# scroll-tech/scroll-prover

Measured on NVIDIA H100. Metric: chunk-proof wall-sec (degree-26 SRS: k=20+24+25 replay), lower is better.
Workload: dtype u32x8 (254-bit Montgomery integers)

## Files before the change

scroll-prover_b200/csrc/msm.cu:

```cuda
#include "common.cuh"
#include "ec.cuh"

namespace b200zk {

static constexpr uint32_t PART_INVALID = 0x1fffffffu;
static constexpr uint32_t PART_GIANT = 0x20000000u;
static constexpr uint32_t PART_STARTS = 0x80000000u;
static constexpr uint32_t PART_ENDS = 0x40000000u;
static constexpr int MSM_MAX_BATCH = 32;
static constexpr int ACC_L_DEFAULT = 256;

struct MsmPlan {
    uint32_t c, W, B;
    uint32_t Ws;
    uint32_t batch;
    uint64_t stride;
    uint64_t NB;
};

struct MsmCols {
    const Fr* p[MSM_MAX_BATCH];
};

__device__ __forceinline__ void ld_affine(const Affine* p, Fq& x, Fq& y) {
// ... 507 lines not shown
__global__ void __launch_bounds__(128) msm_combine_heads(const uint32_t* __restrict__ part_id, const XYZZ* __restrict__ part_val,
                                                         uint64_t nrec, XYZZ* __restrict__ buckets) {
    uint64_t r = (uint64_t)blockIdx.x * blockDim.x + threadIdx.x;
    if (r >= nrec) return;
    uint32_t id = part_id[r];
    if ((id & PART_INVALID) == PART_INVALID || (id & PART_GIANT) || !(id & PART_STARTS)) return;
    XYZZ sum = ld_xyzz(part_val + r);
    uint64_t k = r;
    while (!(id & PART_ENDS)) {
        ++k;
        if (k >= nrec) break;
        id = part_id[k];
        if ((id & PART_INVALID) == PART_INVALID) { id = 0; continue; }
        XYZZ v = ld_xyzz(part_val + k);
        xyzz_add(sum, v);
    }
    st_xyzz(buckets + (part_id[r] & PART_INVALID), sum);
}

static constexpr int COMBINE_LR = 64;
__global__ void __launch_bounds__(128) msm_combine_level(const uint32_t* __restrict__ in_id, const XYZZ* __restrict__ in_val,
                                                         uint64_t nrec, XYZZ* __restrict__ buckets, uint32_t* __restrict__ out_id,
                                                         XYZZ* __restrict__ out_val, uint64_t nthreads,
                                                         const uint32_t* __restrict__ giant_flag) {
    if (*giant_flag == 0) return;
    uint64_t sigma = (uint64_t)blockIdx.x * blockDim.x + threadIdx.x;
    if (sigma >= nthreads) return;
    out_id[2 * sigma] = PART_INVALID;
    out_id[2 * sigma + 1] = PART_INVALID;
    uint64_t r0 = sigma * COMBINE_LR, r1 = r0 + COMBINE_LR;
    if (r1 > nrec) r1 = nrec;
    bool have = false;
    uint32_t cur = 0, flags = 0, slot = 0;
    XYZZ acc = XYZZ::identity();
    auto flush = [&]() {
        if (!have) return;
        if ((flags & PART_STARTS) && (flags & PART_ENDS)) {
            st_xyzz(buckets + cur, acc);
        } else {
            out_id[2 * sigma + slot] = cur | flags | PART_GIANT;
            st_xyzz(out_val + 2 * sigma + slot, acc);
            ++slot;
        }
    };
    for (uint64_t r = r0; r < r1; ++r) {
        uint32_t id = in_id[r];
        if ((id & PART_INVALID) == PART_INVALID || !(id & PART_GIANT)) continue;
        uint32_t bkt = id & PART_INVALID;
        if (!have || bkt != cur) {
            flush();
            have = true;
            cur = bkt;
            flags = id & (PART_STARTS | PART_ENDS);
            acc = ld_xyzz(in_val + r);
        } else {
            flags |= id & (PART_STARTS | PART_ENDS);
            XYZZ v = ld_xyzz(in_val + r);
            xyzz_add(acc, v);
        }
    }
    flush();
}

__global__ void __launch_bounds__(128) msm_combine_final(const uint32_t* __restrict__ part_id, const XYZZ* __restrict__ part_val,
                                                         uint64_t nrec, XYZZ* __restrict__ buckets, const uint32_t* __restrict__ giant_flag) {
    if (*giant_flag == 0) return;
    uint64_t r = (uint64_t)blockIdx.x * blockDim.x + threadIdx.x;
    if (r >= nrec) return;
    uint32_t id = part_id[r];
    if ((id & PART_INVALID) == PART_INVALID || !(id & PART_GIANT) || !(id & PART_STARTS)) return;
    XYZZ sum = ld_xyzz(part_val + r);
    uint64_t k = r;
    while (!(id & PART_ENDS)) {
        ++k;
        if (k >= nrec) break;
        id = part_id[k];
        if ((id & PART_INVALID) == PART_INVALID || !(id & PART_GIANT)) { id = 0; continue; }
        XYZZ v = ld_xyzz(part_val + k);
        xyzz_add(sum, v);
    }
    st_xyzz(buckets + (part_id[r] & PART_INVALID), sum);
}

static constexpr int RED_T = 128;

__device__ __forceinline__ void block_tree_sum(XYZZ& v, XYZZ* sh) {
    st_xyzz(sh + threadIdx.x, v);
    __syncthreads();
    for (uint32_t s = blockDim.x >> 1; s > 0; s >>= 1) {
        if (threadIdx.x < s) {
            XYZZ a = ld_xyzz(sh + threadIdx.x), b = ld_xyzz(sh + threadIdx.x + s);
            xyzz_add(a, b);
            st_xyzz(sh + threadIdx.x, a);
        }
        __syncthreads();
    }
    v = ld_xyzz(sh);
}

__global__ void __launch_bounds__(RED_T, 4) msm_rowcol_sums(const XYZZ* __restrict__ buckets, uint32_t B, uint32_t kc, XYZZ* __restrict__ vec) {
    __shared__ XYZZ sh[RED_T];
    const uint32_t cols = 1u << kc, rows = B >> kc;
    const XYZZ* bk = buckets + (uint64_t)blockIdx.y * B;
    XYZZ acc = XYZZ::identity();
    if (blockIdx.x < rows) {
        const XYZZ* r = bk + (uint64_t)blockIdx.x * cols;
        for (uint32_t lo = threadIdx.x; lo < cols; lo += blockDim.x) {
            XYZZ v = ld_xyzz(r + lo);
            xyzz_add(acc, v);
        }
    } else {
        uint32_t lo = blockIdx.x - rows;
        for (uint32_t hi = threadIdx.x; hi < rows; hi += blockDim.x) {
            XYZZ v = ld_xyzz(bk + (uint64_t)hi * cols + lo);
            xyzz_add(acc, v);
        }
    }
    block_tree_sum(acc, sh);
    if (threadIdx.x == 0) st_xyzz(vec + (uint64_t)blockIdx.y * (rows + cols) + blockIdx.x, acc);
}

__global__ void __launch_bounds__(RED_T, 4) msm_bit_sums(const XYZZ* __restrict__ vec, uint32_t B, uint32_t kc, uint32_t q_max,
                                                         XYZZ* __restrict__ out) {
    __shared__ XYZZ sh[RED_T];
    const uint32_t cols = 1u << kc, rows = B >> kc;
    const uint32_t which = blockIdx.y, b = blockIdx.x;
    const uint32_t m = which == 0 ? rows : cols;
    const XYZZ* v = vec + (uint64_t)blockIdx.z * (rows + cols) + (which == 0 ? 0 : rows);
    XYZZ acc = XYZZ::identity();
    const bool total = (b == q_max);
    if (total ? (which == 0) : ((1u << b) < m)) {
        for (uint32_t j = threadIdx.x; j < m; j += blockDim.x)
            if (total || ((j >> b) & 1u)) {
                XYZZ e = ld_xyzz(v + j);
                xyzz_add(acc, e);
            }
    }
    block_tree_sum(acc, sh);
    if (threadIdx.x == 0) st_xyzz(out + ((uint64_t)blockIdx.z * 2 + which) * (q_max + 1) + b, acc);
}

__global__ void __launch_bounds__(64) msm_finish(MsmPlan pl, uint32_t kc, uint32_t q_max, const XYZZ* __restrict__ bits_all, Jacobian* out_all) {
    __shared__ XYZZ ws[2];
    const uint32_t cols = 1u << kc, rows = pl.B >> kc;
    const uint32_t warp = threadIdx.x >> 5, lane = threadIdx.x & 31;
    Jacobian* out = out_all + blockIdx.x;
    XYZZ acc = XYZZ::identity();
    for (uint32_t w = pl.Ws; w-- > 0;) {
        const uint64_t set = (uint64_t)blockIdx.x * pl.Ws + w;
        const XYZZ* bits = bits_all + set * 2 * (q_max + 1);
        if (lane == 0) {
            const uint32_t m = warp == 0 ? rows : cols;
            const XYZZ* bv = bits + (uint64_t)warp * (q_max + 1);
            XYZZ h = XYZZ::identity();
            uint32_t q = 0;
            while ((1u << q) < m) ++q;
            for (uint32_t b = q; b-- > 0;) {
                if (!h.is_identity()) h = xyzz_dbl(h);
                XYZZ e = ld_xyzz(bv + b);
                xyzz_add(h, e);
            }
            st_xyzz(ws + warp, h);
        }
        __syncthreads();
        if (threadIdx.x == 0) {
            if (!acc.is_identity())
                for (uint32_t d = 0; d < pl.c; ++d) acc = xyzz_dbl(acc);
            XYZZ s = ld_xyzz(ws);
            for (uint32_t d = 0; d < kc; ++d) s = xyzz_dbl(s);
            XYZZ t = ld_xyzz(bits + q_max), u = ld_xyzz(ws + 1);
            xyzz_add(s, t);
            xyzz_add(s, u);
            xyzz_add(acc, s);
        }
        __syncthreads();
    }
    if (threadIdx.x == 0) *out = xyzz_to_jacobian_normalized(acc);
}

__global__ void g1_sum_kernel(const Jacobian* pts, uint64_t count, Jacobian* out) {
    if (threadIdx.x || blockIdx.x) return;
    XYZZ acc = XYZZ::identity();
    for (uint64_t i = 0; i < count; ++i) {
        XYZZ p = xyzz_from_jacobian(pts[i]);
        xyzz_add(acc, p);
    }
    *out = xyzz_to_jacobian_normalized(acc);
}

__global__ void __launch_bounds__(128) g1_generator_mul_kernel(const Fr* scalars, uint64_t n, Affine* out) {
    uint64_t i = (uint64_t)blockIdx.x * blockDim.x + threadIdx.x;
    if (i >= n) return;
    Fr s = scalars[i].from_mont();
    Fq gx = Fq::one(), gy = Fq::one().dbl();
    XYZZ acc = XYZZ::identity();
    for (int limb = 7; limb >= 0; --limb)
        for (int b = 31; b >= 0; --b) {
            acc = xyzz_dbl(acc);
            if ((s.l.v[limb] >> b) & 1) xyzz_madd(acc, gx, gy);
        }
    out[i] = xyzz_to_affine(acc);
}

static uint32_t pick_window(uint64_t n) {
    if (n < 32) return n < 4 ? 2 : 4;
    double best = 1e300;
    uint32_t bc = 8;
    for (uint32_t c = 5; c <= 23; ++c) {
        uint32_t W = 254 / c + 1;
        if ((double)n * W >= 4.0e9) continue;
        double cost = (double)n * W * 10.0 + (double)W * (double)(1ull << c) * 40.0 + (double)W * 4096.0;
        if (cost < best) {
            best = cost;
            bc = c;
        }
    }
    return bc;
}

static size_t align_up(size_t v, size_t a) { return (v + a - 1) / a * a; }

__global__ void __launch_bounds__(128) srs_shift_kernel(const Affine* __restrict__ in, Affine* __restrict__ out, uint64_t n, uint32_t c) {
    uint64_t i = (uint64_t)blockIdx.x * blockDim.x + threadIdx.x;
    if (i >= n) return;
    Affine a = in[i];
    XYZZ p = xyzz_from_affine(a);
    for (uint32_t d = 0; d < c; ++d) p = xyzz_dbl(p);
    out[i] = xyzz_to_affine(p);
}

static uint32_t pick_window_precomputed(uint64_t n) {
    double best = 1e300;
    uint32_t bc = 10;
    for (uint32_t c = 8; c <= 23; ++c) {
        uint32_t W = 254 / c + 1;
        if ((double)n * W >= 2.0e9) continue;
        double cost = (double)n * W * 10.0 + (double)(1ull << c) * 40.0;
        if (cost < best) {
            best = cost;
            bc = c;
        }
    }
    return bc;
}

static int32_t srs_precompute_run(b200zk_ctx* ctx, Affine* tables, uint64_t n, uint32_t c, uint32_t W) {
    for (uint32_t w = 1; w < W; ++w) {
        srs_shift_kernel<<<(uint32_t)((n + 127) / 128), 128, 0, ctx->stream>>>(tables + (uint64_t)(w - 1) * n, tables + (uint64_t)w * n, n, c);
        B2_LAUNCH_CHECK(ctx);
    }
    return B200ZK_OK;
}

static uint32_t msm_max_batch(uint64_t n, uint32_t pre_c) {
    uint32_t c = pre_c ? pre_c : pick_window(n);
    uint64_t per_col = (n ? n : 1) * (254 / c + 1);
    uint64_t b = (1ull << 28) / per_col;
    return (uint32_t)(b < 1 ? 1 : (b > MSM_MAX_BATCH ? MSM_MAX_BATCH : b));
}

static int32_t msm_run_batch(b200zk_ctx* ctx, const Affine* bases, const Fr* const* cols, uint32_t batch, uint64_t n, Jacobian* out_dev,
                             uint32_t pre_c, uint64_t pre_stride) {
    if (n >= (1ull << 31)) return fail(ctx, B200ZK_E_UNSUPPORTED, "msm: n = %llu >= 2^31", (unsigned long long)n);
    if (batch < 1 || batch > (uint32_t)MSM_MAX_BATCH) return fail(ctx, B200ZK_E_INVALID, "msm: batch %u out of range [1,%d]", batch, MSM_MAX_BATCH);
    MsmPlan pl;
    pl.c = pre_c ? pre_c : (ctx->msm_window ? ctx->msm_window : pick_window(n));
    if (pl.c < 2 || pl.c > 24) return fail(ctx, B200ZK_E_INVALID, "msm: window %u out of range [2,24]", pl.c);
    pl.W = 254 / pl.c + 1;
    pl.B = 1u << (pl.c - 1);
    pl.Ws = pre_c ? 1 : pl.W;
    pl.batch = batch;
    pl.stride = pre_c ? pre_stride : 0;
    pl.NB = (uint64_t)batch * pl.Ws * pl.B;
    uint64_t max_entries = n * pl.W * batch;
    if (max_entries >= 0xffffffffull) return fail(ctx, B200ZK_E_UNSUPPORTED, "msm: n*W*batch too large for window %u", pl.c);
    MsmCols colp;
    for (int q = 0; q < MSM_MAX_BATCH; ++q) colp.p[q] = cols[q < (int)batch ? q : 0];
    ctx->last_c = pl.c;
    ctx->last_windows = pl.W;
    ctx->last_adds = n * pl.W;

    const uint32_t ACC_L = ctx->msm_acc_l ? ctx->msm_acc_l : (uint32_t)ACC_L_DEFAULT;
    uint64_t nthreads = (max_entries + ACC_L - 1) / ACC_L;
    if (nthreads == 0) nthreads = 1;
    SortPlan sp;
    sp.FB = pl.c - 1 < SORT_FB_MAX ? pl.c - 1 : SORT_FB_MAX;
    sp.K = pl.B >> sp.FB;
    sp.wpg = pl.Ws == 1 ? pl.W : (COUNT_LOCAL_MAX / sp.K < 1 ? 1 : (COUNT_LOCAL_MAX / sp.K < pl.W ? COUNT_LOCAL_MAX / sp.K : pl.W));
    const uint32_t groups = (pl.W + sp.wpg - 1) / sp.wpg;
    const uint64_t nbins = pl.NB >> sp.FB;
    const uint32_t F = 1u << sp.FB;
    const uint64_t max_big = max_entries / SORT_BIG + 1;
    uint32_t ntiles = (uint32_t)((nbins + SCAN_TILE - 1) / SCAN_TILE);
    size_t off = 0;
    auto carve = [&](size_t bytes) { size_t o = off; off = align_up(off + bytes, 256); return o; };
    size_t o_offs = carve(4 * (pl.NB + 1));
    size_t o_bcnt = carve(4 * (nbins + 1)), o_boff = carve(4 * (nbins + 1)), o_bcur = carve(4 * (nbins + 1));
    size_t o_big = carve(4 * (max_big + 1)), o_bigc = carve(4 * 2 * F * max_big);
    size_t o_tiles = carve(4 * (size_t)(ntiles + 1));
    size_t o_flag = carve(256);
    size_t o_entries = carve(4 * (max_entries + 4));
    size_t o_digits = carve(4 * (max_entries + 4));
    size_t o_buckets = carve(sizeof(XYZZ) * pl.NB);
    size_t pval_bytes = sizeof(XYZZ) * 2 * nthreads;
    size_t o_pid = carve(4 * 2 * nthreads), o_pval = carve(pval_bytes > max_entries + 16 ? pval_bytes : max_entries + 16);
    uint64_t nthreads2 = (2 * nthreads + COMBINE_LR - 1) / COMBINE_LR;
    size_t o_pid2 = carve(4 * 2 * nthreads2), o_pval2 = carve(sizeof(XYZZ) * 2 * nthreads2);
    const uint32_t kc = pl.c / 2;
    const uint32_t red_cols = 1u << kc, red_rows = pl.B >> kc;
    const uint32_t sets = batch * pl.Ws;
    size_t red_len = (size_t)sets * (red_rows + red_cols);
    uint32_t q_max = 0;
    while ((1u << q_max) < (red_rows > red_cols ? red_rows : red_cols)) ++q_max;
    size_t o_gr = carve(sizeof(XYZZ) * red_len), o_sums = carve(sizeof(XYZZ) * 2 * (q_max + 1) * sets);
    B2_TRY(scratch_reserve(ctx, ctx->msm_work, off));
    char* base = (char*)ctx->msm_work.p;
    uint32_t* offsets = (uint32_t*)(base + o_offs);
    uint32_t* bin_cnt = (uint32_t*)(base + o_bcnt);
    uint32_t* bin_off = (uint32_t*)(base + o_boff);
    uint32_t* bin_cur = (uint32_t*)(base + o_bcur);
    uint32_t* big_list = (uint32_t*)(base + o_big);
    uint32_t* big_cnt = (uint32_t*)(base + o_bigc);
    uint32_t* tiles = (uint32_t*)(base + o_tiles);
    uint32_t* giant_flag = (uint32_t*)(base + o_flag);
    uint32_t* staged = (uint32_t*)(base + o_entries);
    uint32_t* digits = (uint32_t*)(base + o_digits);
    uint32_t* entries = digits;
    uint32_t* pid2 = (uint32_t*)(base + o_pid2);
    XYZZ* pval2 = (XYZZ*)(base + o_pval2);
    XYZZ* buckets = (XYZZ*)(base + o_buckets);
    uint32_t* pid = (uint32_t*)(base + o_pid);
    XYZZ* pval = (XYZZ*)(base + o_pval);
    uint8_t* fine = (uint8_t*)(base + o_pval);
    XYZZ* grpR = (XYZZ*)(base + o_gr);
    XYZZ* red_sums = (XYZZ*)(base + o_sums);

    cudaStream_t st = ctx->stream;
    B2_CUDA(ctx, cudaMemsetAsync(bin_cnt, 0, 4 * (nbins + 1), st));
    B2_CUDA(ctx, cudaMemsetAsync(big_list, 0, o_tiles - o_big, st));
    B2_CUDA(ctx, cudaMemsetAsync(giant_flag, 0, 4, st));
    B2_CUDA(ctx, cudaMemsetAsync(buckets, 0, sizeof(XYZZ) * pl.NB, st));
    const size_t count_smem = 4ull * (pl.Ws == 1 ? 1u : sp.wpg) * sp.K;
    const size_t part_smem = sp.K > PART_STAGE_K ? 4ull * sp.K : 4ull * (2 * sp.K + 2 * PART_TILE);
    if (!(ctx->smem_optin & (1u << 9))) {
        const int most = (int)(4 * (1u << (24 - 1 - SORT_FB_MAX)));
        B2_CUDA(ctx, cudaFuncSetAttribute(msm_count, cudaFuncAttributeMaxDynamicSharedMemorySize, most));
        B2_CUDA(ctx, cudaFuncSetAttribute(msm_partition, cudaFuncAttributeMaxDynamicSharedMemorySize, most));
        ctx->smem_optin |= 1u << 9;
    }
    if (n) {
        int per_sm = 1;
        B2_CUDA(ctx, cudaOccupancyMaxActiveBlocksPerMultiprocessor(&per_sm, msm_count, SORT_T, count_smem));
        if (per_sm < 1) per_sm = 1;
        uint64_t want = (n + SORT_T - 1) / SORT_T;
        uint32_t per = ((uint32_t)ctx->sm_count * (uint32_t)per_sm + batch * groups - 1) / (batch * groups);
        uint32_t blocks = (uint32_t)(want < per ? want : per);
        {
            ProfScope ps_(ctx, PROF_MSM_COUNT);
            msm_count<<<dim3(blocks, batch, groups), SORT_T, count_smem, st>>>(colp, n, pl, sp, bin_cnt, digits);
        }
        B2_LAUNCH_CHECK(ctx);
    }
    {
        ProfScope ps_(ctx, PROF_MSM_SCAN);
        scan_tile_sums<<<ntiles, SCAN_TPB, 0, st>>>(bin_cnt, nbins, tiles);
        B2_LAUNCH_CHECK(ctx);
        scan_tile_offsets<<<1, SCAN_TPB, 0, st>>>(tiles, ntiles, offsets + pl.NB, ctx->msm_adds_dev);
        B2_LAUNCH_CHECK(ctx);
        scan_apply<<<ntiles, SCAN_TPB, 0, st>>>(bin_cnt, nbins, tiles, bin_off, bin_cur);
        B2_LAUNCH_CHECK(ctx);
    }
    if (n) {
        {
            ProfScope ps_(ctx, PROF_MSM_SCATTER);
            uint32_t pblocks = (uint32_t)((n + PART_TILE - 1) / PART_TILE);
            msm_partition<<<dim3(pblocks, batch * pl.W), PART_T, part_smem, st>>>(digits, n, pl, sp, bin_cur, staged, fine);
            B2_LAUNCH_CHECK(ctx);
            msm_bin_sort<<<(uint32_t)nbins, SORT_T, 0, st>>>(bin_off, nbins, sp, staged, fine, offsets, entries, big_list);
            B2_LAUNCH_CHECK(ctx);
            uint32_t gblocks = (uint32_t)ctx->sm_count * 2;
            msm_big_count<<<gblocks, SORT_T, 0, st>>>(bin_off, nbins, sp, fine, offsets, big_list, big_cnt);
            B2_LAUNCH_CHECK(ctx);
            msm_big_scatter<<<gblocks, SORT_T, 0, st>>>(bin_off, nbins, sp, staged, fine, offsets, entries, big_list, big_cnt);
        }
        B2_LAUNCH_CHECK(ctx);
        uint32_t ablocks = (uint32_t)((nthreads + 255) / 256);
        {
            ProfScope ps_(ctx, PROF_MSM_ACCUM);
            msm_accumulate<<<ablocks, 256, 0, st>>>(bases, entries, offsets, pl.NB, buckets, pid, pval, nthreads, giant_flag, ACC_L);
        }
        B2_LAUNCH_CHECK(ctx);
        {
            ProfScope ps_(ctx, PROF_MSM_COMBINE);
            uint64_t nrec = 2 * nthreads;
            msm_combine_heads<<<(uint32_t)((nrec + 127) / 128), 128, 0, st>>>(pid, pval, nrec, buckets);
            B2_LAUNCH_CHECK(ctx);
            uint32_t *in_id = pid, *out_id = pid2;
            XYZZ *in_val = pval, *out_val = pval2;
            while (nrec > 2048) {
                uint64_t nt = (nrec + COMBINE_LR - 1) / COMBINE_LR;
                msm_combine_level<<<(uint32_t)((nt + 127) / 128), 128, 0, st>>>(in_id, in_val, nrec, buckets, out_id, out_val, nt, giant_flag);
                B2_LAUNCH_CHECK(ctx);
                nrec = 2 * nt;
                uint32_t* ti = in_id; in_id = out_id; out_id = ti;
                XYZZ* tv = in_val; in_val = out_val; out_val = tv;
            }
            msm_combine_final<<<(uint32_t)((nrec + 127) / 128), 128, 0, st>>>(in_id, in_val, nrec, buckets, giant_flag);
            B2_LAUNCH_CHECK(ctx);
        }
    }
    {
        ProfScope ps_(ctx, PROF_MSM_REDUCE);
        msm_rowcol_sums<<<dim3(red_rows + red_cols, sets), RED_T, 0, st>>>(buckets, pl.B, kc, grpR);
        B2_LAUNCH_CHECK(ctx);
        msm_bit_sums<<<dim3(q_max + 1, 2, sets), RED_T, 0, st>>>(grpR, pl.B, kc, q_max, red_sums);
        B2_LAUNCH_CHECK(ctx);
        msm_finish<<<batch, 64, 0, st>>>(pl, kc, q_max, red_sums, out_dev);
        B2_LAUNCH_CHECK(ctx);
    }
    return B200ZK_OK;
}

int32_t msm_bases(b200zk_ctx* ctx, const Affine* bases, const Fr* scalars, uint64_t n, Jacobian* out_dev) {
    return msm_run_batch(ctx, bases, &scalars, 1, n, out_dev, 0, 0);
}

int32_t srs_init(b200zk_ctx* ctx, b200zk_srs* s, const void* g1_affine) {
    const uint64_t n = s->n;
    s->dev_bases = nullptr;
    s->pre_c = 0;
    s->pre_W = 1;
    size_t bytes = sizeof(Affine) * (n ? n : 1);
    if (ctx->srs_precompute && n >= (1ull << 16)) {
        uint32_t c = pick_window_precomputed(n), W = 254 / c + 1;
        size_t free_b = 0, total_b = 0;
        if (cudaMemGetInfo(&free_b, &total_b) == cudaSuccess && (double)bytes * W < 0.35 * (double)free_b) {
            s->pre_c = c;
            s->pre_W = W;
            bytes *= W;
        }
    }
    cudaError_t e = cudaMalloc(&s->dev_bases, bytes);
    if (e != cudaSuccess) {
        (void)cudaGetLastError();
        s->dev_bases = nullptr;
        return fail(ctx, B200ZK_E_OOM, "srs_register: cudaMalloc(%zu) failed", bytes);
    }
    cudaMemcpyKind kind = is_device_ptr(g1_affine) ? cudaMemcpyDeviceToDevice : cudaMemcpyHostToDevice;
    e = n ? cudaMemcpyAsync(s->dev_bases, g1_affine, sizeof(Affine) * n, kind, ctx->stream) : cudaSuccess;
    if (e == cudaSuccess) e = cudaStreamSynchronize(ctx->stream);
    if (e != cudaSuccess) {
        srs_free(s);
        return fail(ctx, B200ZK_E_CUDA, "srs_register: upload failed: %s", cudaGetErrorString(e));
    }
    if (s->pre_c) {
        int32_t rc = srs_precompute_run(ctx, (Affine*)s->dev_bases, n, s->pre_c, s->pre_W);
        if (rc == B200ZK_OK && cudaStreamSynchronize(ctx->stream) != cudaSuccess) rc = B200ZK_E_CUDA;
        if (rc != B200ZK_OK) {
            srs_free(s);
            return fail(ctx, rc, "srs_register: precomputation failed");
        }
    }
    return B200ZK_OK;
}

void srs_free(b200zk_srs* s) {
    if (s->dev_bases) cudaFree(s->dev_bases);
    s->dev_bases = nullptr;
}

static uint32_t srs_pre_c(const b200zk_srs* s, uint64_t n) { return (s->pre_c && n * 16 >= s->n) ? s->pre_c : 0; }

uint32_t msm_srs_max_batch(const b200zk_srs* s, uint64_t n) { return msm_max_batch(n, srs_pre_c(s, n)); }

int32_t msm_srs(b200zk_ctx* ctx, const b200zk_srs* s, uint64_t first, const Fr* const* cols, uint32_t count, uint64_t n,
                Jacobian* out_dev) {
    const uint32_t pre_c = srs_pre_c(s, n), bmax = msm_max_batch(n, pre_c);
    const Affine* bases = (const Affine*)s->dev_bases + first;
    for (uint32_t j = 0; j < count; j += bmax)
        B2_TRY(msm_run_batch(ctx, bases, cols + j, count - j < bmax ? count - j : bmax, n, out_dev + j, pre_c, s->n));
    return B200ZK_OK;
}

int32_t g1_sum_run(b200zk_ctx* ctx, const Jacobian* pts, uint64_t count, Jacobian* out_dev) {
    g1_sum_kernel<<<1, 32, 0, ctx->stream>>>(pts, count, out_dev);
    B2_LAUNCH_CHECK(ctx);
    return B200ZK_OK;
}

int32_t g1_generator_mul_run(b200zk_ctx* ctx, const Fr* scalars, uint64_t n, Affine* out) {
    if (!n) return B200ZK_OK;
    g1_generator_mul_kernel<<<(uint32_t)((n + 127) / 128), 128, 0, ctx->stream>>>(scalars, n, out);
    B2_LAUNCH_CHECK(ctx);
    return B200ZK_OK;
}

}
```

scroll-prover_b200/csrc/ntt.cu:

```cuda
#include "common.cuh"

namespace b200zk {

static constexpr int NTT_THREADS = 256;
static constexpr int NTT_MAX_DIGIT = 8;

struct Fr3 {
    Fr c[3];
};

struct NttPass {
    uint32_t log_n, P, p;
    uint32_t dig[4];
    uint32_t t;
    uint32_t m;
    uint32_t rest;
    uint32_t log_in;
    int pre, post;
};

__device__ __forceinline__ Fr sel3(const Fr3& t, uint32_t r) {
    Fr o;
#pragma unroll
    for (int i = 0; i < 8; ++i) o.l.v[i] = r == 0 ? t.c[0].l.v[i] : (r == 1 ? t.c[1].l.v[i] : t.c[2].l.v[i]);
    return o;
}

struct LevelRoots {
    Fr w[29];
};

__device__ __forceinline__ Fr ld_fr(const Fr* p) {
    const uint4* q = reinterpret_cast<const uint4*>(p);
    uint4 a = q[0], b = q[1];
    Fr r;
    r.l.v[0] = a.x; r.l.v[1] = a.y; r.l.v[2] = a.z; r.l.v[3] = a.w;
    r.l.v[4] = b.x; r.l.v[5] = b.y; r.l.v[6] = b.z; r.l.v[7] = b.w;
    return r;
}
__device__ __forceinline__ Fr ldg_fr(const Fr* p) {
    const uint4* q = reinterpret_cast<const uint4*>(p);
    uint4 a = __ldg(q), b = __ldg(q + 1);
    Fr r;
    r.l.v[0] = a.x; r.l.v[1] = a.y; r.l.v[2] = a.z; r.l.v[3] = a.w;
    r.l.v[4] = b.x; r.l.v[5] = b.y; r.l.v[6] = b.z; r.l.v[7] = b.w;
    return r;
}
__device__ __forceinline__ void st_fr(Fr* p, const Fr& r) {
    uint4* q = reinterpret_cast<uint4*>(p);
    q[0] = make_uint4(r.l.v[0], r.l.v[1], r.l.v[2], r.l.v[3]);
    q[1] = make_uint4(r.l.v[4], r.l.v[5], r.l.v[6], r.l.v[7]);
}
struct PartTw {
    const Fr* etab;
    uint32_t j, log_N;
};

__device__ __forceinline__ Fr ext_pow(const PartTw& pt, uint32_t e) {
    const uint32_t half = 1u << (pt.log_N - 1);
    Fr w = ldg_fr(pt.etab + (e & (half - 1)));
    return e >= half ? Fr::zero() - w : w;
}

__device__ __forceinline__ Fr ld_sm(const uint4* lo, const uint4* hi, uint32_t i) {
    uint4 a = lo[i], b = hi[i];
    Fr r;
    r.l.v[0] = a.x; r.l.v[1] = a.y; r.l.v[2] = a.z; r.l.v[3] = a.w;
    r.l.v[4] = b.x; r.l.v[5] = b.y; r.l.v[6] = b.z; r.l.v[7] = b.w;
    return r;
}
__device__ __forceinline__ void st_sm(uint4* lo, uint4* hi, uint32_t i, const Fr& r) {
    lo[i] = make_uint4(r.l.v[0], r.l.v[1], r.l.v[2], r.l.v[3]);
    hi[i] = make_uint4(r.l.v[4], r.l.v[5], r.l.v[6], r.l.v[7]);
}

__global__ void ntt_build_table(Fr* tab, LevelRoots roots, uint32_t log_n) {
    uint64_t e = (uint64_t)blockIdx.x * blockDim.x + threadIdx.x;
    uint64_t total = 1ull << log_n;
    if (e >= total) return;
    if (e == 0) {
        st_fr(tab, Fr::one());
        return;
    }
    uint32_t u = 64 - __clzll(e);
    uint32_t j = (uint32_t)(e - (1ull << (u - 1)));
    Fr base = roots.w[u], acc = Fr::one();
    while (j) {
        if (j & 1) acc = acc * base;
        base = base.sqr();
        j >>= 1;
    }
    st_fr(tab + e, acc);
}

template <int C, bool LAST, bool PART>
__global__ void __launch_bounds__(NTT_THREADS, 3)
ntt_pass_kernel(const Fr* __restrict__ in, Fr* __restrict__ out, const Fr* __restrict__ tab, NttPass ps, Fr3 pre_c,
                Fr3 post_c, PartTw pt) {
    extern __shared__ uint4 smem[];
    const uint32_t m = ps.m, L = 1u << m, E = L * C;
    uint4* lo = smem;
    uint4* hi = smem + E;
    uint4* twlo = hi + E;
    uint4* twhi = twlo + L;
    const uint32_t tid = threadIdx.x, NT = blockDim.x;
    const uint32_t t = ps.t, rest = ps.rest, n = ps.log_n;
    const uint32_t swz_shift = (C == 8 && m >= 3) ? (m - 3) : 31;
    auto idx = [&](uint32_t pos, uint32_t lane) -> uint32_t {
        if (C == 8) return pos * C + (lane ^ ((pos >> swz_shift) & 7u));
        return pos;
    };

    uint64_t base;
    uint32_t c;
    uint64_t rowstride = 0;
    if (!LAST) {
        uint32_t groups_log = rest - 3;
        uint64_t tile = blockIdx.x;
        uint64_t o = tile >> groups_log, g = tile & ((1ull << groups_log) - 1);
        base = (o << (n - t)) + g * C;
        uint32_t sh = t, tq = 0;
        c = 0;
        for (uint32_t q = 0; q < ps.p; ++q) {
            sh -= ps.dig[q];
            uint32_t kq = (uint32_t)(o >> sh) & ((1u << ps.dig[q]) - 1);
            c |= kq << tq;
            tq += ps.dig[q];
        }
    } else {
        c = blockIdx.x * C;
        uint32_t tq = 0;
        uint64_t pos = 0;
        for (uint32_t q = 0; q + 1 < ps.P; ++q) {
            uint32_t kq = (c >> tq) & ((1u << ps.dig[q]) - 1);
            tq += ps.dig[q];
            pos |= (uint64_t)kq << (n - tq);
        }
        base = pos;
        rowstride = (ps.P > 1) ? (1ull << (n - ps.dig[0])) : 0;
    }

    const uint64_t in_len = 1ull << ps.log_in;
    const bool zskip = (ps.p == 0) && (ps.log_in + 2 == n) && (m >= 2);
    const uint32_t E_load = zskip ? (E >> 2) : E, L_load = zskip ? (L >> 2) : L;
    for (uint32_t e = tid; e < E_load; e += NT) {
        uint32_t lane, d;
        uint64_t gi;
        if (!LAST) {
            lane = e % C;
            d = e / C;
            gi = base + ((uint64_t)d << rest) + lane;
        } else {
            d = e & (L_load - 1);
            lane = e / L_load;
            gi = base + lane * rowstride + d;
        }
        Fr v;
        if (ps.p == 0 && gi >= in_len) {
            v = Fr::zero();
        } else {
            v = ld_fr(in + gi);
            if (ps.p == 0 && ps.pre) {
                uint32_t r3 = (uint32_t)(gi % 3);
                if (r3) v = v * sel3(pre_c, r3);
                if (PART) {
                    uint32_t e = pt.j * (uint32_t)gi;
                    if (e) v = v * ext_pow(pt, e);
                }
            }
        }
        uint32_t pos = __brev(d) >> (32 - m);
        if (zskip) {
#pragma unroll
            for (uint32_t r = 0; r < 4; ++r) st_sm(lo, hi, idx(pos + r, lane), v);
        } else {
            st_sm(lo, hi, idx(pos, lane), v);
        }
    }
    if (!LAST) {
        for (uint32_t j = tid; j < L; j += NT) {
            if (j == 0) continue;
            uint32_t s = 32 - __clz(j);
            uint32_t K = j - (1u << (s - 1));
            uint64_t src = (1ull << (t + s - 1)) + ((uint64_t)K << t) + c;
            Fr w = ldg_fr(tab + src);
            st_sm(twlo, twhi, j, w);
        }
    }
    __syncthreads();

    auto twiddle = [&](uint32_t s, uint32_t K, uint32_t lane, Fr& w) -> bool {
        if (!LAST) {
            if (K == 0 && c == 0) return false;
            w = ld_sm(twlo, twhi, (1u << (s - 1)) + K);
            return true;
        }
        uint64_t j = ((uint64_t)K << t) + c + lane;
        if (j == 0) return false;
        w = ldg_fr(tab + (1ull << (t + s - 1)) + j);
        return true;
    };
    uint32_t s = zskip ? 3 : 1;
    for (; s + 1 <= m; s += 2) {
        const uint32_t h = 1u << (s - 1);
        const uint32_t ng = (L >> 2) * C;
        for (uint32_t q = tid; q < ng; q += NT) {
            uint32_t lane = q % C, gq = q / C;
            uint32_t K = gq & (h - 1), blk = gq >> (s - 1);
            uint32_t p = (blk << (s + 1)) + K;
            uint32_t i0 = idx(p, lane), i1 = idx(p + h, lane), i2 = idx(p + 2 * h, lane), i3 = idx(p + 3 * h, lane);
            Fr a = ld_sm(lo, hi, i0), b = ld_sm(lo, hi, i1), cc = ld_sm(lo, hi, i2), d = ld_sm(lo, hi, i3);
            Fr w;
            if (twiddle(s, K, lane, w)) {
                b = b * w;
                d = d * w;
            }
            Fr a1 = a + b, b1 = a - b, c1 = cc + d, d1 = cc - d;
            if (twiddle(s + 1, K, lane, w)) c1 = c1 * w;
            twiddle(s + 1, K + h, lane, w);
            d1 = d1 * w;
            st_sm(lo, hi, i0, a1 + c1);
            st_sm(lo, hi, i2, a1 - c1);
            st_sm(lo, hi, i1, b1 + d1);
            st_sm(lo, hi, i3, b1 - d1);
        }
        __syncthreads();
    }
    if (s == m) {
        const uint32_t half = 1u << (s - 1);
        const uint32_t nb = (L >> 1) * C;
        for (uint32_t b = tid; b < nb; b += NT) {
            uint32_t lane = b % C, bb = b / C;
            uint32_t K = bb & (half - 1), blk = bb >> (s - 1);
            uint32_t p0 = (blk << s) + K, p1 = p0 + half;
            uint32_t i0 = idx(p0, lane), i1 = idx(p1, lane);
            Fr u = ld_sm(lo, hi, i0), v = ld_sm(lo, hi, i1), w;
            if (twiddle(s, K, lane, w)) v = v * w;
            st_sm(lo, hi, i0, u + v);
            st_sm(lo, hi, i1, u - v);
        }
        __syncthreads();
    }

    for (uint32_t e = tid; e < E; e += NT) {
        uint32_t lane = e % C, K = e / C;
        Fr v = ld_sm(lo, hi, idx(K, lane));
        uint64_t go;
        if (!LAST) {
            go = base + ((uint64_t)K << rest) + lane;
        } else {
            go = ((uint64_t)K << t) + c + lane;
            if (ps.post) {
                v = v * sel3(post_c, (uint32_t)(go % 3));
                if (PART) {
                    uint32_t e = (0u - pt.j * (uint32_t)go) & ((1u << pt.log_N) - 1);
                    if (e) v = v * ext_pow(pt, e);
                }
            }
        }
        st_fr(out + go, v);
    }
}

static Fr host_halve(const Fr& x) {
    Fr r = x;
    uint32_t carry = 0;
    if (x.l.v[0] & 1) {
        uint32_t m[8];
        Fr::modulus(m);
        carry = leaf::add8(r.l.v, x.l.v, m);
    }
    for (int i = 0; i < 8; ++i) {
        uint32_t nxt = (i < 7) ? r.l.v[i + 1] : carry;
        r.l.v[i] = (r.l.v[i] >> 1) | (nxt << 31);
    }
    return r;
}

Fr host_zeta() {
    Fr z;
    const uint32_t v[8] = {0x55fcd653u, 0x0363f299u, 0x5fc1e200u, 0x73e7950bu,
                           0x576d9d24u, 0xc5fce83eu, 0xa1c3a4d4u, 0x059c805du};
    for (int i = 0; i < 8; ++i) z.l.v[i] = v[i];
    return z;
}

int32_t ntt_get_table(b200zk_ctx* ctx, const Fr& omega, uint32_t log_n, const Fr** out) {
    LevelRoots roots;
    roots.w[log_n] = omega;
    for (uint32_t u = log_n; u > 0; --u) roots.w[u - 1] = roots.w[u].sqr();
    Fr minus_one = Fr::zero() - Fr::one();
    if (!(roots.w[0] == Fr::one()) || (log_n >= 1 && !(roots.w[1] == minus_one)))
        return fail(ctx, B200ZK_E_INVALID, "omega is not a primitive 2^%u-th root of unity", log_n);
    for (auto& tt : ctx->tables) {
        if (tt.log_n < log_n) continue;
        Fr w = tt.omega;
        for (uint32_t i = tt.log_n; i > log_n; --i) w = w.sqr();
        if (w == omega) {
            *out = tt.dev;
            return B200ZK_OK;
        }
    }
    for (size_t i = 0; i < ctx->tables.size(); ++i) {
        Fr w = omega;
        bool same = false;
        if (ctx->tables[i].log_n < log_n) {
            for (uint32_t k = log_n; k > ctx->tables[i].log_n; --k) w = w.sqr();
            same = (w == ctx->tables[i].omega);
        }
        if (same) {
            B2_CUDA(ctx, cudaStreamSynchronize(ctx->stream));
            B2_CUDA(ctx, cudaFree(ctx->tables[i].dev));
            ctx->tables.erase(ctx->tables.begin() + i);
            break;
        }
    }
    for (uint32_t u = log_n + 1; u < 29; ++u) roots.w[u] = Fr::one();
    Fr* dev = nullptr;
    size_t bytes = sizeof(Fr) << log_n;
    cudaError_t e = cudaMalloc(&dev, bytes);
    if (e != cudaSuccess) {
        (void)cudaGetLastError();
        return fail(ctx, B200ZK_E_OOM, "twiddle table cudaMalloc(%zu) failed", bytes);
    }
    uint64_t total = 1ull << log_n;
    uint32_t tpb = 256;
    uint32_t blocks = (uint32_t)((total + tpb - 1) / tpb);
    {
        ProfScope ps(ctx, PROF_NTT_TABLE);
        ntt_build_table<<<blocks, tpb, 0, ctx->stream>>>(dev, roots, log_n);
    }
    B2_LAUNCH_CHECK(ctx);
    ctx->tables.push_back({omega, log_n, dev});
    *out = dev;
    return B200ZK_OK;
}

static void plan_digits(uint32_t log_n, uint32_t* P, uint32_t dig[4]) {
    if (log_n <= NTT_MAX_DIGIT) {
        *P = 1;
        dig[0] = log_n;
        dig[1] = dig[2] = dig[3] = 0;
        return;
    }
    uint32_t p = (log_n + NTT_MAX_DIGIT - 1) / NTT_MAX_DIGIT;
    *P = p;
    uint32_t basebits = log_n / p, extra = log_n % p;
    for (uint32_t i = 0; i < 4; ++i) dig[i] = (i < p) ? basebits + (i < extra ? 1 : 0) : 0;
}

template <int C, bool LAST, bool PART>
static int32_t launch_pass(b200zk_ctx* ctx, const Fr* in, Fr* out, const Fr* tab, const NttPass& ps, const Fr3& pre_c,
                           const Fr3& post_c, const PartTw& pt) {
    uint32_t L = 1u << ps.m, E = L * C;
    size_t smem = (size_t)(2 * E + (LAST ? 0 : 2 * L)) * sizeof(uint4);
    const uint32_t optin_bit = 1u << ((C == 8 ? 0 : 2) + (LAST ? 1 : 0) + (PART ? 4 : 0));
    if (!(ctx->smem_optin & optin_bit)) {
        B2_CUDA(ctx, cudaFuncSetAttribute(ntt_pass_kernel<C, LAST, PART>, cudaFuncAttributeMaxDynamicSharedMemorySize,
                                          (int)((2 * (1u << NTT_MAX_DIGIT) * C + 2 * (1u << NTT_MAX_DIGIT)) * sizeof(uint4))));
        ctx->smem_optin |= optin_bit;
    }
    uint64_t tiles = (1ull << ps.log_n) / E;
    uint32_t nb = (L >> 2) * C;
    uint32_t threads = nb >= NTT_THREADS ? NTT_THREADS : (nb < 32 ? 32 : nb);
    {
        ProfScope psc(ctx, PROF_NTT_PASS);
        ntt_pass_kernel<C, LAST, PART><<<(uint32_t)tiles, threads, smem, ctx->stream>>>(in, out, tab, ps, pre_c, post_c, pt);
    }
    B2_LAUNCH_CHECK(ctx);
    return B200ZK_OK;
}

template <bool PART>
static int32_t ntt_run_impl(b200zk_ctx* ctx, const Fr* in, uint32_t log_in, Fr* out, uint32_t log_n, const Fr& omega,
                            int inverse_scale, int coset_mode, const PartTw& pt, const Fr& extra_scale) {
    if (log_n > 28) return fail(ctx, B200ZK_E_INVALID, "log_n %u exceeds Fr two-adicity 28", log_n);
    if (log_in > log_n) return fail(ctx, B200ZK_E_INVALID, "log_in %u > log_n %u", log_in, log_n);
    if (coset_mode < 0 || coset_mode > 2) return fail(ctx, B200ZK_E_INVALID, "bad coset_mode %d", coset_mode);
    if (log_n == 0 && !PART) {
        if (in != out) B2_CUDA(ctx, cudaMemcpyAsync(out, in, sizeof(Fr), cudaMemcpyDeviceToDevice, ctx->stream));
        return B200ZK_OK;
    }
    const Fr* tab = nullptr;
    B2_TRY(ntt_get_table(ctx, omega, log_n, &tab));

    Fr zeta = host_zeta(), zeta2 = zeta.sqr();
    Fr3 pre_c, post_c;
    pre_c.c[0] = Fr::one();
    pre_c.c[1] = zeta;
    pre_c.c[2] = zeta2;
    Fr scale = extra_scale;
    if (inverse_scale)
        for (uint32_t i = 0; i < log_n; ++i) scale = host_halve(scale);
    post_c.c[0] = scale;
    post_c.c[1] = (coset_mode == B200ZK_COSET_POST) ? scale * zeta2 : scale;
    post_c.c[2] = (coset_mode == B200ZK_COSET_POST) ? scale * zeta : scale;

    NttPass ps;
    memset(&ps, 0, sizeof ps);
    ps.log_n = log_n;
    plan_digits(log_n, &ps.P, ps.dig);
    const int pre = (coset_mode == B200ZK_COSET_PRE), post = (inverse_scale || coset_mode == B200ZK_COSET_POST);

    if (ps.P == 1) {
        ps.p = 0;
        ps.t = 0;
        ps.m = log_n;
        ps.rest = 0;
        ps.log_in = log_in;
        ps.pre = pre;
        ps.post = post;
        return launch_pass<1, true, PART>(ctx, in, out, tab, ps, pre_c, post_c, pt);
    }
    size_t bytes = sizeof(Fr) << log_n;
    B2_TRY(scratch_reserve(ctx, ctx->ntt_work, bytes));
    Fr* W = (Fr*)ctx->ntt_work.p;
    uint32_t t = 0;
    for (uint32_t p = 0; p < ps.P; ++p) {
        ps.p = p;
        ps.t = t;
        ps.m = ps.dig[p];
        ps.rest = log_n - t - ps.m;
        ps.log_in = (p == 0) ? log_in : log_n;
        ps.pre = (p == 0) ? pre : 0;
        ps.post = (p + 1 == ps.P) ? post : 0;
        if (p + 1 < ps.P)
            B2_TRY((launch_pass<8, false, PART>(ctx, p == 0 ? in : W, W, tab, ps, pre_c, post_c, pt)));
        else
            B2_TRY((launch_pass<8, true, PART>(ctx, W, out, tab, ps, pre_c, post_c, pt)));
        t += ps.m;
    }
    return B200ZK_OK;
}

int32_t ntt_run(b200zk_ctx* ctx, const Fr* in, uint32_t log_in, Fr* out, uint32_t log_n, const Fr& omega,
                int inverse_scale, int coset_mode) {
    return ntt_run_impl<false>(ctx, in, log_in, out, log_n, omega, inverse_scale, coset_mode, PartTw{nullptr, 0, 0}, Fr::one());
}

int32_t ntt_run_part(b200zk_ctx* ctx, const Fr* in, Fr* out, uint32_t k, uint32_t log_N, const Fr& ext_omega, uint32_t part,
                     bool inverse, const Fr& scale) {
    if (log_N <= k || log_N > 28 || part >= (1u << (log_N - k)))
// ... 14 lines not shown
```

Measured before the change: 4.212.

## Replace row/column bit-sum bucket reduction with hierarchical segmented running sums

Replaces the three-kernel bucket reduction (row/column sums, per-bit sums, serial finish) with a multi-level segmented running-sum scheme. Each thread computes a running sum over a contiguous bucket segment, and the segment totals and partial sums are combined in further levels until one sum per window remains. The reduction scratch buffer is placed inside the staged-entries region when it fits. This is meant to give more parallelism and less redundant point addition in the reduce phase, at the cost of extra kernel launches per level and per-thread shared-memory accumulators.

```diff
diff --git a/scroll-prover_b200/csrc/msm.cu b/scroll-prover_b200/csrc/msm.cu
--- a/scroll-prover_b200/csrc/msm.cu
+++ b/scroll-prover_b200/csrc/msm.cu
@@ -613,100 +613,51 @@
     st_xyzz(buckets + (part_id[r] & PART_INVALID), sum);
 }
 
-static constexpr int RED_T = 128;
-
-__device__ __forceinline__ void block_tree_sum(XYZZ& v, XYZZ* sh) {
-    st_xyzz(sh + threadIdx.x, v);
-    __syncthreads();
-    for (uint32_t s = blockDim.x >> 1; s > 0; s >>= 1) {
-        if (threadIdx.x < s) {
-            XYZZ a = ld_xyzz(sh + threadIdx.x), b = ld_xyzz(sh + threadIdx.x + s);
-            xyzz_add(a, b);
-            st_xyzz(sh + threadIdx.x, a);
-        }
-        __syncthreads();
-    }
-    v = ld_xyzz(sh);
-}
-
-__global__ void __launch_bounds__(RED_T, 4) msm_rowcol_sums(const XYZZ* __restrict__ buckets, uint32_t B, uint32_t kc, XYZZ* __restrict__ vec) {
-    __shared__ XYZZ sh[RED_T];
-    const uint32_t cols = 1u << kc, rows = B >> kc;
-    const XYZZ* bk = buckets + (uint64_t)blockIdx.y * B;
-    XYZZ acc = XYZZ::identity();
-    if (blockIdx.x < rows) {
-        const XYZZ* r = bk + (uint64_t)blockIdx.x * cols;
-        for (uint32_t lo = threadIdx.x; lo < cols; lo += blockDim.x) {
-            XYZZ v = ld_xyzz(r + lo);
-            xyzz_add(acc, v);
-        }
-    } else {
-        uint32_t lo = blockIdx.x - rows;
-        for (uint32_t hi = threadIdx.x; hi < rows; hi += blockDim.x) {
-            XYZZ v = ld_xyzz(bk + (uint64_t)hi * cols + lo);
-            xyzz_add(acc, v);
-        }
-    }
-    block_tree_sum(acc, sh);
-    if (threadIdx.x == 0) st_xyzz(vec + (uint64_t)blockIdx.y * (rows + cols) + blockIdx.x, acc);
-}
-
-__global__ void __launch_bounds__(RED_T, 4) msm_bit_sums(const XYZZ* __restrict__ vec, uint32_t B, uint32_t kc, uint32_t q_max,
-                                                         XYZZ* __restrict__ out) {
-    __shared__ XYZZ sh[RED_T];
-    const uint32_t cols = 1u << kc, rows = B >> kc;
-    const uint32_t which = blockIdx.y, b = blockIdx.x;
-    const uint32_t m = which == 0 ? rows : cols;
-    const XYZZ* v = vec + (uint64_t)blockIdx.z * (rows + cols) + (which == 0 ? 0 : rows);
-    XYZZ acc = XYZZ::identity();
-    const bool total = (b == q_max);
-    if (total ? (which == 0) : ((1u << b) < m)) {
-        for (uint32_t j = threadIdx.x; j < m; j += blockDim.x)
-            if (total || ((j >> b) & 1u)) {
-                XYZZ e = ld_xyzz(v + j);
-                xyzz_add(acc, e);
-            }
-    }
-    block_tree_sum(acc, sh);
-    if (threadIdx.x == 0) st_xyzz(out + ((uint64_t)blockIdx.z * 2 + which) * (q_max + 1) + b, acc);
-}
-
-__global__ void __launch_bounds__(64) msm_finish(MsmPlan pl, uint32_t kc, uint32_t q_max, const XYZZ* __restrict__ bits_all, Jacobian* out_all) {
-    __shared__ XYZZ ws[2];
-    const uint32_t cols = 1u << kc, rows = pl.B >> kc;
-    const uint32_t warp = threadIdx.x >> 5, lane = threadIdx.x & 31;
-    Jacobian* out = out_all + blockIdx.x;
+static constexpr int RED_T = 128, RED_BLOCKS = 4;
+static constexpr uint32_t RED_UP_LG = 2;
+
+template <bool UP>
+__global__ void __launch_bounds__(RED_T, RED_BLOCKS) msm_seg_sums(const XYZZ* __restrict__ V, const XYZZ* __restrict__ U, uint32_t m, uint32_t lgL,
+                                                         uint64_t nthreads, XYZZ* __restrict__ R_out, XYZZ* __restrict__ P_out) {
+    __shared__ XYZZ acc_sh[RED_T];
+    const uint64_t g = (uint64_t)blockIdx.x * blockDim.x + threadIdx.x;
+    if (g >= nthreads) return;
+    const uint32_t L = 1u << lgL, T = m >> lgL;
+    const uint64_t set = g / T, t = g - set * T;
+    const uint64_t base = set * m + t * L;
+    XYZZ* acc = acc_sh + threadIdx.x;
+    XYZZ R = XYZZ::identity();
+    st_xyzz(acc, R);
+    for (uint32_t j = L; j-- > 0;) {
+        XYZZ a = ld_xyzz(acc);
+        xyzz_add(a, R);
+        if (UP) {
+            XYZZ u = ld_xyzz(U + base + j);
+            xyzz_add(a, u);
+        }
+        st_xyzz(acc, a);
+        XYZZ v = ld_xyzz(V + base + j);
+        xyzz_add(R, v);
+    }
+    XYZZ p = ld_xyzz(acc);
+    if (!UP) xyzz_add(p, R);
+    st_xyzz(P_out + g, p);
+    if (T > 1) {
+        for (uint32_t d = 0; d < lgL; ++d) R = xyzz_dbl(R);
+        st_xyzz(R_out + g, R);
+    }
+}
+
+__global__ void __launch_bounds__(32) msm_finish(MsmPlan pl, const XYZZ* __restrict__ sums, Jacobian* out) {
+    const uint32_t col = blockIdx.x * blockDim.x + threadIdx.x;
+    if (col >= pl.batch) return;
     XYZZ acc = XYZZ::identity();
     for (uint32_t w = pl.Ws; w-- > 0;) {
-        const uint64_t set = (uint64_t)blockIdx.x * pl.Ws + w;
-        const XYZZ* bits = bits_all + set * 2 * (q_max + 1);
-        if (lane == 0) {
-            const uint32_t m = warp == 0 ? rows : cols;
-            const XYZZ* bv = bits + (uint64_t)warp * (q_max + 1);
-            XYZZ h = XYZZ::identity();
-            uint32_t q = 0;
-            while ((1u << q) < m) ++q;
-            for (uint32_t b = q; b-- > 0;) {
-                if (!h.is_identity()) h = xyzz_dbl(h);
-                XYZZ e = ld_xyzz(bv + b);
-                xyzz_add(h, e);
-            }
-            st_xyzz(ws + warp, h);
-        }
-        __syncthreads();
-        if (threadIdx.x == 0) {
-            if (!acc.is_identity())
-                for (uint32_t d = 0; d < pl.c; ++d) acc = xyzz_dbl(acc);
-            XYZZ s = ld_xyzz(ws);
-            for (uint32_t d = 0; d < kc; ++d) s = xyzz_dbl(s);
-            XYZZ t = ld_xyzz(bits + q_max), u = ld_xyzz(ws + 1);
-            xyzz_add(s, t);
-            xyzz_add(s, u);
-            xyzz_add(acc, s);
-        }
-        __syncthreads();
-    }
-    if (threadIdx.x == 0) *out = xyzz_to_jacobian_normalized(acc);
+        for (uint32_t d = 0; d < pl.c && !acc.is_identity(); ++d) acc = xyzz_dbl(acc);
+        XYZZ s = ld_xyzz(sums + (uint64_t)col * pl.Ws + w);
+        xyzz_add(acc, s);
+    }
+    out[col] = xyzz_to_jacobian_normalized(acc);
 }
 
 __global__ void g1_sum_kernel(const Jacobian* pts, uint64_t count, Jacobian* out) {
@@ -837,13 +788,14 @@
     size_t o_pid = carve(4 * 2 * nthreads), o_pval = carve(pval_bytes > max_entries + 16 ? pval_bytes : max_entries + 16);
     uint64_t nthreads2 = (2 * nthreads + COMBINE_LR - 1) / COMBINE_LR;
     size_t o_pid2 = carve(4 * 2 * nthreads2), o_pval2 = carve(sizeof(XYZZ) * 2 * nthreads2);
-    const uint32_t kc = pl.c / 2;
-    const uint32_t red_cols = 1u << kc, red_rows = pl.B >> kc;
     const uint32_t sets = batch * pl.Ws;
-    size_t red_len = (size_t)sets * (red_rows + red_cols);
-    uint32_t q_max = 0;
-    while ((1u << q_max) < (red_rows > red_cols ? red_rows : red_cols)) ++q_max;
-    size_t o_gr = carve(sizeof(XYZZ) * red_len), o_sums = carve(sizeof(XYZZ) * 2 * (q_max + 1) * sets);
+    const uint64_t red_target = (uint64_t)ctx->sm_count * RED_T * RED_BLOCKS;
+    uint32_t lgT1 = 0;
+    while ((1ull << (lgT1 + 1)) * sets <= red_target && (1u << (lgT1 + 1)) <= pl.B / 2) ++lgT1;
+    const uint32_t T1 = 1u << lgT1, T2 = lgT1 > RED_UP_LG ? T1 >> RED_UP_LG : 1u;
+    const size_t red_a = sizeof(XYZZ) * 2 * (size_t)sets * T1, red_b = sizeof(XYZZ) * 2 * (size_t)sets * T2;
+    const bool red_in_staged = align_up(red_a, 256) + red_b <= 4 * (max_entries + 4);
+    const size_t o_red = red_in_staged ? o_entries : carve(align_up(red_a, 256) + red_b);
     B2_TRY(scratch_reserve(ctx, ctx->msm_work, off));
     char* base = (char*)ctx->msm_work.p;
     uint32_t* offsets = (uint32_t*)(base + o_offs);
@@ -863,8 +815,7 @@
     uint32_t* pid = (uint32_t*)(base + o_pid);
     XYZZ* pval = (XYZZ*)(base + o_pval);
     uint8_t* fine = (uint8_t*)(base + o_pval);
-    XYZZ* grpR = (XYZZ*)(base + o_gr);
-    XYZZ* red_sums = (XYZZ*)(base + o_sums);
+    XYZZ* red_buf[2] = {(XYZZ*)(base + o_red), (XYZZ*)(base + o_red + align_up(red_a, 256))};
 
     cudaStream_t st = ctx->stream;
     B2_CUDA(ctx, cudaMemsetAsync(bin_cnt, 0, 4 * (nbins + 1), st));
@@ -940,13 +891,36 @@
             B2_LAUNCH_CHECK(ctx);
         }
     }
+    const XYZZ* sums = nullptr;
     {
         ProfScope ps_(ctx, PROF_MSM_REDUCE);
-        msm_rowcol_sums<<<dim3(red_rows + red_cols, sets), RED_T, 0, st>>>(buckets, pl.B, kc, grpR);
-        B2_LAUNCH_CHECK(ctx);
-        msm_bit_sums<<<dim3(q_max + 1, 2, sets), RED_T, 0, st>>>(grpR, pl.B, kc, q_max, red_sums);
-        B2_LAUNCH_CHECK(ctx);
-        msm_finish<<<batch, 64, 0, st>>>(pl, kc, q_max, red_sums, out_dev);
+        const XYZZ *V = buckets, *U = nullptr;
+        uint32_t m = pl.B, lgL = pl.c - 1 - lgT1;
+        for (int lvl = 0;; ++lvl) {
+            const uint32_t T = m >> lgL;
+            const uint64_t nt = (uint64_t)sets * T;
+            XYZZ* R = red_buf[lvl & 1];
+            XYZZ* P = R + nt;
+            const uint32_t blocks = (uint32_t)((nt + RED_T - 1) / RED_T);
+            if (U)
+                msm_seg_sums<true><<<blocks, RED_T, 0, st>>>(V, U, m, lgL, nt, R, P);
+            else
+                msm_seg_sums<false><<<blocks, RED_T, 0, st>>>(V, U, m, lgL, nt, R, P);
+            B2_LAUNCH_CHECK(ctx);
+            if (T == 1) {
+                sums = P;
+                break;
+            }
+            V = R;
+            U = P;
+            m = T;
+            lgL = 0;
+            while (lgL < RED_UP_LG && (2u << lgL) <= m) ++lgL;
+        }
+    }
+    {
+        ProfScope ps_(ctx, PROF_MSM_FINISH);
+        msm_finish<<<(batch + 31) / 32, 32, 0, st>>>(pl, sums, out_dev);
         B2_LAUNCH_CHECK(ctx);
     }
     return B200ZK_OK;
```

Measured after the change: 4.149, median of 6. 1.02x faster.

## Stage NTT inputs and per-lane twiddles into shared memory via cp.async

Applied to the files above, without the earlier changes.

Non-first NTT passes now load their inputs with cp.async straight into shared memory, and twiddles are also staged asynchronously. The LAST pass now keeps a per-lane twiddle table in shared memory instead of reading global memory inside every butterfly. To keep that larger shared-memory footprint bounded, the last digit is capped at 7 bits, which can raise the number of passes for some sizes. It also unrolls the digit loops and reorders the radix-4 butterfly to lower register pressure.

```diff
diff --git a/scroll-prover_b200/csrc/ntt.cu b/scroll-prover_b200/csrc/ntt.cu
--- a/scroll-prover_b200/csrc/ntt.cu
+++ b/scroll-prover_b200/csrc/ntt.cu
@@ -4,6 +4,7 @@
 
 static constexpr int NTT_THREADS = 256;
 static constexpr int NTT_MAX_DIGIT = 8;
+static constexpr int NTT_MAX_LAST_DIGIT = 7;
 
 struct Fr3 {
     Fr c[3];
@@ -93,16 +94,24 @@
     st_fr(tab + e, acc);
 }
 
+__device__ __forceinline__ void cp_async_fr(uint4* lo, uint4* hi, uint32_t i, const Fr* src) {
+    const uint4* q = reinterpret_cast<const uint4*>(src);
+    asm volatile("cp.async.cg.shared.global [%0], [%1], 16;\n" ::"r"((uint32_t)__cvta_generic_to_shared(lo + i)), "l"(q));
+    asm volatile("cp.async.cg.shared.global [%0], [%1], 16;\n" ::"r"((uint32_t)__cvta_generic_to_shared(hi + i)), "l"(q + 1));
+}
+__device__ __forceinline__ void cp_async_wait() { asm volatile("cp.async.wait_all;\n" ::: "memory"); }
+
 template <int C, bool LAST, bool PART>
 __global__ void __launch_bounds__(NTT_THREADS, 3)
 ntt_pass_kernel(const Fr* __restrict__ in, Fr* __restrict__ out, const Fr* __restrict__ tab, NttPass ps, Fr3 pre_c,
                 Fr3 post_c, PartTw pt) {
     extern __shared__ uint4 smem[];
+    constexpr uint32_t CT = LAST ? C : 1;
     const uint32_t m = ps.m, L = 1u << m, E = L * C;
     uint4* lo = smem;
     uint4* hi = smem + E;
     uint4* twlo = hi + E;
-    uint4* twhi = twlo + L;
+    uint4* twhi = twlo + L * CT;
     const uint32_t tid = threadIdx.x, NT = blockDim.x;
     const uint32_t t = ps.t, rest = ps.rest, n = ps.log_n;
     const uint32_t swz_shift = (C == 8 && m >= 3) ? (m - 3) : 31;
@@ -121,7 +130,9 @@
         base = (o << (n - t)) + g * C;
         uint32_t sh = t, tq = 0;
         c = 0;
-        for (uint32_t q = 0; q < ps.p; ++q) {
+#pragma unroll
+        for (uint32_t q = 0; q < 3; ++q) {
+            if (q >= ps.p) break;
             sh -= ps.dig[q];
             uint32_t kq = (uint32_t)(o >> sh) & ((1u << ps.dig[q]) - 1);
             c |= kq << tq;
@@ -131,13 +142,22 @@
         c = blockIdx.x * C;
         uint32_t tq = 0;
         uint64_t pos = 0;
-        for (uint32_t q = 0; q + 1 < ps.P; ++q) {
+#pragma unroll
+        for (uint32_t q = 0; q < 3; ++q) {
+            if (q + 1 >= ps.P) break;
             uint32_t kq = (c >> tq) & ((1u << ps.dig[q]) - 1);
             tq += ps.dig[q];
             pos |= (uint64_t)kq << (n - tq);
         }
         base = pos;
         rowstride = (ps.P > 1) ? (1ull << (n - ps.dig[0])) : 0;
+    }
+
+    for (uint32_t e = tid + CT; e < L * CT; e += NT) {
+        const uint32_t j = e / CT, col = e % CT;
+        const uint32_t s = 32 - __clz(j);
+        const uint32_t K = j - (1u << (s - 1));
+        cp_async_fr(twlo, twhi, e, tab + (1ull << (t + s - 1)) + ((uint64_t)K << t) + c + col);
     }
 
     const uint64_t in_len = 1ull << ps.log_in;
@@ -155,12 +175,17 @@
             lane = e / L_load;
             gi = base + lane * rowstride + d;
         }
+        uint32_t pos = __brev(d) >> (32 - m);
+        if (ps.p != 0) {
+            cp_async_fr(lo, hi, idx(pos, lane), in + gi);
+            continue;
+        }
         Fr v;
-        if (ps.p == 0 && gi >= in_len) {
+        if (gi >= in_len) {
             v = Fr::zero();
         } else {
             v = ld_fr(in + gi);
-            if (ps.p == 0 && ps.pre) {
+            if (ps.pre) {
                 uint32_t r3 = (uint32_t)(gi % 3);
                 if (r3) v = v * sel3(pre_c, r3);
                 if (PART) {
@@ -169,7 +194,6 @@
                 }
             }
         }
-        uint32_t pos = __brev(d) >> (32 - m);
         if (zskip) {
 #pragma unroll
             for (uint32_t r = 0; r < 4; ++r) st_sm(lo, hi, idx(pos + r, lane), v);
@@ -177,27 +201,13 @@
             st_sm(lo, hi, idx(pos, lane), v);
         }
     }
-    if (!LAST) {
-        for (uint32_t j = tid; j < L; j += NT) {
-            if (j == 0) continue;
-            uint32_t s = 32 - __clz(j);
-            uint32_t K = j - (1u << (s - 1));
-            uint64_t src = (1ull << (t + s - 1)) + ((uint64_t)K << t) + c;
-            Fr w = ldg_fr(tab + src);
-            st_sm(twlo, twhi, j, w);
-        }
-    }
+    cp_async_wait();
     __syncthreads();
 
     auto twiddle = [&](uint32_t s, uint32_t K, uint32_t lane, Fr& w) -> bool {
-        if (!LAST) {
-            if (K == 0 && c == 0) return false;
-            w = ld_sm(twlo, twhi, (1u << (s - 1)) + K);
-            return true;
-        }
-        uint64_t j = ((uint64_t)K << t) + c + lane;
-        if (j == 0) return false;
-        w = ldg_fr(tab + (1ull << (t + s - 1)) + j);
+        const uint32_t col = LAST ? lane : 0;
+        if ((K | (c + col)) == 0) return false;
+        w = ld_sm(twlo, twhi, ((1u << (s - 1)) + K) * CT + col);
         return true;
     };
     uint32_t s = zskip ? 3 : 1;
@@ -209,18 +219,25 @@
             uint32_t K = gq & (h - 1), blk = gq >> (s - 1);
             uint32_t p = (blk << (s + 1)) + K;
             uint32_t i0 = idx(p, lane), i1 = idx(p + h, lane), i2 = idx(p + 2 * h, lane), i3 = idx(p + 3 * h, lane);
-            Fr a = ld_sm(lo, hi, i0), b = ld_sm(lo, hi, i1), cc = ld_sm(lo, hi, i2), d = ld_sm(lo, hi, i3);
-            Fr w;
-            if (twiddle(s, K, lane, w)) {
-                b = b * w;
-                d = d * w;
+            Fr w, a1, b1;
+            {
+                Fr a = ld_sm(lo, hi, i0), b = ld_sm(lo, hi, i1);
+                if (twiddle(s, K, lane, w)) b = b * w;
+                a1 = a + b;
+                b1 = a - b;
             }
-            Fr a1 = a + b, b1 = a - b, c1 = cc + d, d1 = cc - d;
+            Fr c1, d1;
+            {
+                Fr cc = ld_sm(lo, hi, i2), d = ld_sm(lo, hi, i3);
+                if (twiddle(s, K, lane, w)) d = d * w;
+                c1 = cc + d;
+                d1 = cc - d;
+            }
             if (twiddle(s + 1, K, lane, w)) c1 = c1 * w;
+            st_sm(lo, hi, i0, a1 + c1);
+            st_sm(lo, hi, i2, a1 - c1);
             twiddle(s + 1, K + h, lane, w);
             d1 = d1 * w;
-            st_sm(lo, hi, i0, a1 + c1);
-            st_sm(lo, hi, i2, a1 - c1);
             st_sm(lo, hi, i1, b1 + d1);
             st_sm(lo, hi, i3, b1 - d1);
         }
@@ -343,7 +360,7 @@
         dig[1] = dig[2] = dig[3] = 0;
         return;
     }
-    uint32_t p = (log_n + NTT_MAX_DIGIT - 1) / NTT_MAX_DIGIT;
+    uint32_t p = 1 + (log_n - NTT_MAX_LAST_DIGIT + NTT_MAX_DIGIT - 1) / NTT_MAX_DIGIT;
     *P = p;
     uint32_t basebits = log_n / p, extra = log_n % p;
     for (uint32_t i = 0; i < 4; ++i) dig[i] = (i < p) ? basebits + (i < extra ? 1 : 0) : 0;
@@ -352,12 +369,16 @@
 template <int C, bool LAST, bool PART>
 static int32_t launch_pass(b200zk_ctx* ctx, const Fr* in, Fr* out, const Fr* tab, const NttPass& ps, const Fr3& pre_c,
                            const Fr3& post_c, const PartTw& pt) {
+    constexpr uint32_t CT = LAST ? C : 1;
+    constexpr uint32_t max_m = (LAST && C > 1) ? NTT_MAX_LAST_DIGIT : NTT_MAX_DIGIT;
+    if (ps.m > max_m) return fail(ctx, B200ZK_E_INVALID, "NTT pass digit %u exceeds %u", ps.m, max_m);
+    auto smem_bytes = [](uint32_t m) { return (size_t)(2 * (C << m) + 2 * (CT << m)) * sizeof(uint4); };
     uint32_t L = 1u << ps.m, E = L * C;
-    size_t smem = (size_t)(2 * E + (LAST ? 0 : 2 * L)) * sizeof(uint4);
+    size_t smem = smem_bytes(ps.m);
     const uint32_t optin_bit = 1u << ((C == 8 ? 0 : 2) + (LAST ? 1 : 0) + (PART ? 4 : 0));
     if (!(ctx->smem_optin & optin_bit)) {
         B2_CUDA(ctx, cudaFuncSetAttribute(ntt_pass_kernel<C, LAST, PART>, cudaFuncAttributeMaxDynamicSharedMemorySize,
-                                          (int)((2 * (1u << NTT_MAX_DIGIT) * C + 2 * (1u << NTT_MAX_DIGIT)) * sizeof(uint4))));
+                                          (int)smem_bytes(max_m)));
         ctx->smem_optin |= optin_bit;
     }
     uint64_t tiles = (1ull << ps.log_n) / E;
```

Measured after the change: 4.210 before, 4.161 after, median of 6. 1.01x faster.
